# PeterouZh/CIPS-3Dplusplus

Hardware: AMD Instinct MI355X
Metric: rendered views/sec at FFHQ 1024^2 (generator forward: 64x64-ray NeRF + StyleGAN2 decoder) (higher is better)
Workload: dtype f32 (split-fp16 MFMA products x3, f32 accumulate and storage); 1 GPU; ffhq_r1024_nerf64x64x24_D2_B1_fp32; img_size=64, n_samples=24, N_layers_renderer=2, resolution=1024, parallelism=views x1, views_in_flight=2

## Files before the change

### cips_3dplusplus_amd/csrc/decoder.hip

```cpp
#include <stdlib.h>

#include <type_traits>

#include "common.h"

namespace {

typedef float f32x16 __attribute__((ext_vector_type(16)));
typedef float f32x4 __attribute__((ext_vector_type(4)));
typedef short s16x4 __attribute__((ext_vector_type(4)));
typedef _Float16 h8 __attribute__((ext_vector_type(8)));

typedef _Float16 h4 __attribute__((ext_vector_type(4)));
typedef _Float16 h2 __attribute__((ext_vector_type(2)));
__device__ __forceinline__ float pack_split(float x) { return __uint_as_float(cips3d_split_word(x)); }
__device__ __forceinline__ float pack_split(float x, float k) { return __uint_as_float(cips3d_split_word(x, k)); }
__device__ __forceinline__ void unpack_frag(float p0, float p1, float p2, float p3, h4& hi, h4& lo) {
  typedef unsigned u32x2_t __attribute__((ext_vector_type(2)));
  const unsigned a0 = __float_as_uint(p0), a1 = __float_as_uint(p1), a2 = __float_as_uint(p2), a3 = __float_as_uint(p3);
  hi = __builtin_bit_cast(h4, u32x2_t{__builtin_amdgcn_perm(a1, a0, 0x05040100u), __builtin_amdgcn_perm(a3, a2, 0x05040100u)});
  lo = __builtin_bit_cast(h4, u32x2_t{__builtin_amdgcn_perm(a1, a0, 0x07060302u), __builtin_amdgcn_perm(a3, a2, 0x07060302u)});
}
__device__ __forceinline__ void split_frag(float v0, float v1, float v2, float v3, h4& hi, h4& lo) {
  typedef unsigned u32x2_t __attribute__((ext_vector_type(2)));
// ... 889 lines not shown
          o.x += sv.x; o.y += sv.y; o.z += sv.z; o.w += sv.w;
        }
      }
      *reinterpret_cast<float4*>(out + ((int64_t)b * 3 + c) * HW + qq * 4) = o;
    }
  }
}

__global__ void __launch_bounds__(256) torgb_scalar_kernel(const float* __restrict__ x, const float* __restrict__ wm,
                                                           const float* __restrict__ bias, const float* __restrict__ skip,
                                                           int skip_up, const float* __restrict__ fir,
                                                           float* __restrict__ out, int B, int Cin, int H, int W) {
  const int64_t HW = (int64_t)H * W;
  const int64_t total = (int64_t)B * HW;
  for (int64_t idx = (int64_t)blockIdx.x * blockDim.x + threadIdx.x; idx < total; idx += (int64_t)gridDim.x * blockDim.x) {
    const int b = (int)(idx / HW);
    const int64_t n = idx % HW;
    const float* xb = x + (int64_t)b * Cin * HW + n;
    const float* w = wm + (int64_t)b * 3 * Cin;
    float acc[3] = {0.f, 0.f, 0.f};
    for (int i = 0; i < Cin; ++i) {
      const float v = xb[(int64_t)i * HW];
      acc[0] = fmaf(w[i], v, acc[0]); acc[1] = fmaf(w[Cin + i], v, acc[1]); acc[2] = fmaf(w[2 * Cin + i], v, acc[2]);
    }
    const int oy = (int)(n / W), ox = (int)(n % W);
#pragma unroll
    for (int c = 0; c < 3; ++c) {
      float o = acc[c] + bias[c];
      if (skip) {
        if (skip_up) o += up2_tap(skip + ((int64_t)b * 3 + c) * (H / 2) * (W / 2), H / 2, W / 2, oy, ox, fir);
        else o += skip[((int64_t)b * 3 + c) * HW + n];
      }
      out[((int64_t)b * 3 + c) * HW + n] = o;
    }
  }
}

__global__ void __launch_bounds__(256) modconv_kxk_kernel(const float* __restrict__ x, const float* __restrict__ wm,
                                                          float* __restrict__ out, int B, int Cin, int Cout, int H,
                                                          int W, int k, int transpose2, int OH, int OW) {
  const int64_t total = (int64_t)B * Cout * OH * OW;
  const int pad = k / 2;
  for (int64_t idx = (int64_t)blockIdx.x * blockDim.x + threadIdx.x; idx < total;
       idx += (int64_t)gridDim.x * blockDim.x) {
    int64_t t = idx;
    const int ox = (int)(t % OW); t /= OW;
    const int oy = (int)(t % OH); t /= OH;
    const int o = (int)(t % Cout);
    const int b = (int)(t / Cout);
    const float* wrow = wm + ((int64_t)b * Cout + o) * Cin * k * k;
    const float* xb = x + (int64_t)b * Cin * H * W;
    float acc = 0.f;
    for (int i = 0; i < Cin; ++i) {
      const float* xi = xb + (int64_t)i * H * W;
      const float* wi = wrow + i * k * k;
      for (int ky = 0; ky < k; ++ky) {
        int iy;
        if (transpose2) { const int ty = oy - ky; if (ty < 0 || (ty & 1)) continue; iy = ty >> 1; }
        else iy = oy + ky - pad;
        if (iy < 0 || iy >= H) continue;
        for (int kx = 0; kx < k; ++kx) {
          int ix;
          if (transpose2) { const int tx = ox - kx; if (tx < 0 || (tx & 1)) continue; ix = tx >> 1; }
          else ix = ox + kx - pad;
          if (ix < 0 || ix >= W) continue;
          acc = fmaf(xi[(int64_t)iy * W + ix], wi[ky * k + kx], acc);
        }
      }
    }
    out[idx] = acc;
  }
}

struct FusedArgs {
  const float* y_lo; const float* fir; const float* noise1; int64_t nbs1; const float* nw1; const float* bias1;
  const float* wm2; const float* noise2; int64_t nbs2; const float* nw2; const float* bias2; float* out2;
  const float* wm_rgb; const float* bias_rgb; const float* skip; int skip_up; float* rgb;
  int B, H, W;
  int bf16;
  const float* wm_next; float* y_next;
  const float* x_amax; const float* lconst1; const float* lconst2; float* next_amax;
  float next_gain;
  int flat;
};

#ifndef CIPS3D_C128_LATE
#define CIPS3D_C128_LATE true
#endif
#ifndef CIPS3D_C64_MINW
#define CIPS3D_C64_MINW 4
#endif
#ifndef CIPS3D_C32_MINW
#define CIPS3D_C32_MINW 8
#endif
#ifndef CIPS3D_FUSED_AB
#define CIPS3D_FUSED_AB 0
#endif
#ifdef CIPS3D_FUSED_STAMPS
__device__ unsigned long long g_fused_stamps[4][8];
#define FSTAMP(i) do { const unsigned long long t_ = __builtin_amdgcn_s_memtime(); fst_[i] += t_ - ftp_; ftp_ = t_; } while (0)
#define FSTAMP_FLUSH() do { if (tid == 0 && (blockIdx.x & 31) == 0) {    constexpr int sl_ = C == 32 ? 0 : C == 64 ? 1 : C == 128 ? 2 : 3; \
    for (int i_ = 0; i_ < 7; ++i_) atomicAdd(&g_fused_stamps[sl_][i_], fst_[i_]); atomicAdd(&g_fused_stamps[sl_][7], 1ull); } } while (0)
#else
#define FSTAMP(i)
#define FSTAMP_FLUSH()
#endif

template <int C, int WM, int WGM, int WGN, int RW, int BK, int MINW, int PREC, bool NEXT = false, bool XPREF = false,
          bool LATE_OPS = false, bool FLAT = false>
__global__ void __launch_bounds__(64 * WGM * WGN, MINW) fused_up_conv_kernel(FusedArgs a) {
  constexpr bool BF16 = PREC == 1 || PREC == 2;
  constexpr bool YB = PREC == 2;
  constexpr bool SPLIT = PREC == 3;
  typedef typename std::conditional<YB, bf16_t, float>::type ylo_t;
  constexpr int NT = 64 * WGM * WGN;
  constexpr int CW = 64 / RW, TH = RW * WGN, TW = CW, BN = TH * TW;
  constexpr int NSTAGE = C / BK, NBUF = NSTAGE > 1 ? 2 : 1, KQ = BK / 16;
  constexpr int LPR = CW / 4;
  static_assert((WGM * WGN == 8 || WGM * WGN == 4) && 16 * WM * WGM == C && TH % 2 == 0 && C % BK == 0, "tile shape");
  constexpr int NBLK = (TH / 2) * (TW / 4);
  constexpr int BPT = BK * NBLK / NT;
  static_assert((BK * NBLK) % NT == 0 && BPT >= 1, "block split");
  __shared__ __attribute__((aligned(16))) float sB[NBUF * BK * BN];
  __shared__ __attribute__((aligned(16))) float s_nz1[BN + 8];
  __shared__ __attribute__((aligned(16))) float s_red_own[NEXT ? WGM * 3 * BN : 4];
  float* s_red = NEXT ? s_red_own : sB;
  __shared__ __attribute__((aligned(16))) float s_wrgb[3 * C];

  const int tid = threadIdx.x;
#ifdef CIPS3D_FUSED_STAMPS
  unsigned long long fst_[7] = {0, 0, 0, 0, 0, 0, 0}, ftp_ = __builtin_amdgcn_s_memtime();
#endif
  const int wave = __builtin_amdgcn_readfirstlane(tid >> 6);
  const int lane = tid & 63;
  const int wm_i = wave / WGN, wn_i = wave % WGN;
  const int q = lane >> 4, jn = lane & 15;
  const int lrow = jn / LPR, lx4 = jn % LPR;
  const int nloc = (wn_i * RW + lrow) * TW + lx4 * 4;
  const int b = blockIdx.z;
  const int H = a.H, W = a.W, OH = FLAT ? H : 2 * H, OW = FLAT ? W : 2 * W;
  const int tiles_x = OW / TW;
  int bid = blockIdx.x;
  if ((gridDim.x & 7) == 0) bid = (bid & 7) * (gridDim.x >> 3) + (bid >> 3);
  const int ox0 = (bid % tiles_x) * TW, oy0 = (bid / tiles_x) * TH;
  const int HWlo = H * W, HWo = OH * OW;
  const int oy = oy0 + wn_i * RW + lrow, ox = ox0 + lx4 * 4;

  float kact1 = 1.41421356237309515f, k2in = kSplitInv, kact2 = 1.41421356237309515f, kback2 = 1.f, kyn = kSplitInv;

#ifndef CIPS3D_FUSED_TILE_DMA
#define CIPS3D_FUSED_TILE_DMA 1
#endif
  constexpr bool TILE_DMA = CIPS3D_FUSED_TILE_DMA != 0;
  float nw1_u = 0.f;
  float c10_u = 0.f, c11_u = 0.f, c20_u = 0.f, c21a_u = 0.f, c21b_u = 0.f;
  if constexpr (SPLIT && TILE_DMA) {
    if (a.x_amax && !(CIPS3D_FUSED_AB & 1)) {
      const float* l1 = a.lconst1 + b * 4;
      c10_u = l1[0]; c11_u = l1[1];
      if (NEXT) {
        const float* l2 = a.lconst2 + b * 4;
        c20_u = l2[0]; c21a_u = l2[1]; c21b_u = l2[2];
      }
    }
  }
  const float* ab = a.wm2 + (int64_t)b * C * C;
  f32x4 afr_next[KQ][WM];
#pragma unroll
  for (int kq = 0; kq < KQ; ++kq)
#pragma unroll
    for (int i = 0; i < WM; ++i)
      afr_next[kq][i] = *reinterpret_cast<const f32x4*>(ab + (((wm_i * WM + i) * (C / 16) + kq) * 256 + lane * 4));
  constexpr bool LATE = LATE_OPS;
  f32x4 nz2 = {0.f, 0.f, 0.f, 0.f};
  float nw2_u = 0.f;
  f32x4 bias4[WM];
  auto load_epilogue_ops = [&]() {
    if (a.noise2 && a.nw2 && !(CIPS3D_FUSED_AB & 128)) {
      nz2 = *reinterpret_cast<const f32x4*>(a.noise2 + (int64_t)b * a.nbs2 + (oy * OW + ox));
      nw2_u = a.nw2[0];
    }
#pragma unroll
    for (int i = 0; i < WM; ++i) bias4[i] = *reinterpret_cast<const f32x4*>(a.bias2 + (wm_i * WM + i) * 16 + 4 * q);
  };
  if (!LATE) load_epilogue_ops();

  float kf[16];
#pragma unroll
  for (int i = 0; i < 16; ++i) kf[i] = FLAT ? 0.f : a.fir[15 - i];
  const bool rgb_lane = a.wm_rgb && wm_i == 0 && q < 3;
  float skp[3][4];
  f32x4 skv = {0.f, 0.f, 0.f, 0.f};
  float rgb_bias = 0.f;
// ... 472 lines not shown
#pragma unroll
      for (int t = 0; t < OTN; ++t)
#pragma unroll
        for (int c = 0; c < 4; ++c) {
          const f32x4 pv4 = *reinterpret_cast<const f32x4*>(sp + (t * 4 + c) * 256);
#pragma unroll
          for (int r = 0; r < 4; ++r) accn[t][c][r] += pv4[r];
        }
    }
    ylo_t* yn = reinterpret_cast<ylo_t*>(a.y_next) + (int64_t)b * (C / 2) * HWo + (oy * OW + ox);
#pragma unroll
    for (int t = 0; t < OTN; ++t)
#pragma unroll
      for (int r = 0; r < 4; ++r) {
        const float ys = SPLIT ? kyn : 1.f;
        const f32x4 yv = {accn[t][0][r] * ys, accn[t][1][r] * ys, accn[t][2][r] * ys, accn[t][3][r] * ys};
        mxn = fmaxf(fmaxf(fmaxf(fabsf(yv[0]), fabsf(yv[1])), fmaxf(fabsf(yv[2]), fabsf(yv[3]))), mxn);
        if constexpr (YB) cips3d_store_wt8(yn + (t * 16 + 4 * q + r) * HWo, pack_bf16(yv[0], yv[1], yv[2], yv[3]));
        else cips3d_store_wt16(yn + (t * 16 + 4 * q + r) * HWo, yv);
      }
  }
  if (NEXT && !XCHG && a.next_amax && !(a.next_gain > 0.f) && !(CIPS3D_FUSED_AB & 2)) {
    const float m = cips3d_workgroup_max(mxn, s_nz1, wave, lane, WGM * WGN);
    if (tid == 0) cips3d_amax_raise_if(a.next_amax + b * CIPS3D_AMAX_FLOATS, m, blockIdx.x);
  }
  FSTAMP(5);
  if (!a.wm_rgb) { FSTAMP_FLUSH(); return; }
  if (rgb_lane) {
    const int ch = q;
    f32x4 v = {0.f, 0.f, 0.f, 0.f};
#pragma unroll
    for (int m = 0; m < WGM; ++m) {
      const f32x4 t = *reinterpret_cast<const f32x4*>(s_red + (m * 3 + ch) * BN + nloc);
#pragma unroll
      for (int c = 0; c < 4; ++c) v[c] += t[c];
    }
#pragma unroll
    for (int c = 0; c < 4; ++c) v[c] += rgb_bias;
    if (a.skip) {
      if (!FLAT && (a.skip_up & 1)) {
        float so[2][4];
        up2_fir(skp, kf, so);
        const int py = oy & 1;
#pragma unroll
        for (int c = 0; c < 4; ++c) v[c] += py ? so[1][c] : so[0][c];
      } else {
#pragma unroll
        for (int c = 0; c < 4; ++c) v[c] += skv[c];
      }
    }
    if (a.skip_up & 2) {
      unsigned pk = 0;
#pragma unroll
      for (int c = 0; c < 4; ++c) {
        const float cl = fminf(fmaxf(v[c], -1.f), 1.f);
        pk |= (unsigned)__float2int_rn((cl + 1.f) * 127.5f) << (8 * c);
      }
      *reinterpret_cast<unsigned*>(reinterpret_cast<unsigned char*>(a.rgb) + (int64_t)b * 3 * HWo + (ch * HWo + oy * OW + ox)) = pk;
    } else {
      cips3d_store_wt16(a.rgb + (int64_t)b * 3 * HWo + (ch * HWo + oy * OW + ox), v);
    }
  }
  FSTAMP(6);
  FSTAMP_FLUSH();
}

template <int C, int WM, int WGM, int WGN, int RW, int BK, int MINW, bool NEXT, bool XPREF, bool LATE, bool FLAT>
int launch_fused_as(const FusedArgs& a, hipStream_t st) {
  constexpr int TH = RW * WGN, TW = 64 / RW;
  const int up = FLAT ? 1 : 2;
  dim3 grid((unsigned)((up * a.W / TW) * (up * a.H / TH)), 1, (unsigned)a.B);
  if (a.bf16 == 3) hipLaunchKernelGGL((fused_up_conv_kernel<C, WM, WGM, WGN, RW, BK, MINW, 3, NEXT, XPREF, LATE, FLAT>), grid, dim3(64 * WGM * WGN), 0, st, a);
  else if (a.bf16 == 2) hipLaunchKernelGGL((fused_up_conv_kernel<C, WM, WGM, WGN, RW, BK, MINW, 2, NEXT, XPREF, LATE, FLAT>), grid, dim3(64 * WGM * WGN), 0, st, a);
  else if (a.bf16) hipLaunchKernelGGL((fused_up_conv_kernel<C, WM, WGM, WGN, RW, BK, MINW, 1, NEXT, XPREF, LATE, FLAT>), grid, dim3(64 * WGM * WGN), 0, st, a);
  else hipLaunchKernelGGL((fused_up_conv_kernel<C, WM, WGM, WGN, RW, BK, MINW, 0, NEXT, XPREF, LATE, FLAT>), grid, dim3(64 * WGM * WGN), 0, st, a);
  return cips3d_launch_status();
}
template <int C, int WM, int WGM, int WGN, int RW, int BK, int MINW, bool NEXT = false, bool XPREF = false, bool LATE = false>
int launch_fused(const FusedArgs& a, hipStream_t st) {
  return a.flat ? launch_fused_as<C, WM, WGM, WGN, RW, BK, MINW, NEXT, XPREF, LATE, true>(a, st)
                : launch_fused_as<C, WM, WGM, WGN, RW, BK, MINW, NEXT, XPREF, LATE, false>(a, st);
}

}

#ifdef CIPS3D_FUSED_STAMPS
extern "C" int cips3d_debug_read_fused_stamps(unsigned long long* out32) {
  hipDeviceSynchronize();
  hipMemcpyFromSymbol(out32, HIP_SYMBOL(g_fused_stamps), 256);
  unsigned long long z[32] = {0};
  hipMemcpyToSymbol(HIP_SYMBOL(g_fused_stamps), z, 256);
  return 0;
}
#endif

extern "C" int cips3d_modulate_weights(const float* W, const float* s, int64_t s_stride, float* wm, int B, int Cout,
                                       int Cin, int ksq, float scale, int demodulate, void* stream) {
  if (!W || !s || !wm || B < 0 || Cout <= 0 || Cin <= 0 || ksq <= 0) return CIPS3D_E_BADARG;
  if (B == 0) return 0;
  const int packed = (demodulate & 2) ? (((demodulate & 4) ? 2 : 1) | (demodulate & 248)) : 0;
  if ((packed & 32) && (ksq != 1 || (packed & 24))) return CIPS3D_E_UNSUPP;
  if ((packed & 64) && (ksq != 1 || (packed & 63) != 1)) return CIPS3D_E_UNSUPP;
  if (packed && ksq == 1 && (Cout % 32 != 0 || Cin % 8 != 0)) return CIPS3D_E_UNSUPP;
  if ((packed & 16) && ksq == 1 && ((packed & 7) != 1 || Cin % 32 != 0)) return CIPS3D_E_UNSUPP;
  if ((packed & 16) && ksq != 1 && (ksq != 9 || (packed & ~8) != 17)) return CIPS3D_E_UNSUPP;
  if ((packed & 128) && (ksq != 1 || (packed & 127) != 1 || Cin % 32 != 0)) return CIPS3D_E_UNSUPP;
  if (packed && ksq != 1 && (ksq != 9 || (packed & 7) != 1 || Cout % 16 != 0 || Cin % 16 != 0)) return CIPS3D_E_UNSUPP;
  const int64_t rows = (int64_t)B * Cout;
  hipLaunchKernelGGL(modulate_kernel, dim3((unsigned)ceil_div<int64_t>(rows, 4)), dim3(256), 0, as_stream(stream), W,
                     s, s_stride, wm, B, Cout, Cin, ksq, scale, demodulate & 1, packed);
  return cips3d_launch_status();
}

extern "C" int cips3d_modulate_table(const cips3d_modulate_desc* table_dev, int n_desc, int total_rows, int B, float noise_bound,
                                     void* stream) {
  if (!table_dev || n_desc <= 0 || total_rows <= 0 || B < 0 || !(noise_bound >= 0.f)) return CIPS3D_E_BADARG;
  if (B == 0) return 0;
  hipLaunchKernelGGL(modulate_table_kernel, dim3((unsigned)ceil_div(total_rows, 4), (unsigned)B), dim3(256), 0,
                     as_stream(stream), table_dev, n_desc, total_rows, noise_bound);
  return cips3d_launch_status();
}

__global__ void __launch_bounds__(256) split_words_kernel(const float* __restrict__ x, float k, unsigned* __restrict__ words,
                                                          unsigned* __restrict__ pairs, int64_t n) {
  const float ku = cips3d_uniform(k);
  for (int64_t i = (int64_t)blockIdx.x * 256 + threadIdx.x; i < n / 2; i += (int64_t)gridDim.x * 256) {
    words[2 * i] = cips3d_split_word(x[2 * i], ku);
    words[2 * i + 1] = cips3d_split_word(x[2 * i + 1] * k);
    cips3d_split_pair(x[2 * i], x[2 * i + 1], pairs[2 * i], pairs[2 * i + 1]);
  }
}

extern "C" int cips3d_split_words(const float* x, float k, uint32_t* words, uint32_t* pairs, int64_t n, void* stream) {
  if (!x || !words || !pairs || n <= 0 || (n & 1)) return CIPS3D_E_BADARG;
  int64_t blocks = ceil_div<int64_t>(n / 2, 256);
  if (blocks > 4096) blocks = 4096;
  hipLaunchKernelGGL(split_words_kernel, dim3((unsigned)blocks), dim3(256), 0, as_stream(stream), x, k, words, pairs, n);
  return cips3d_launch_status();
}

extern "C" int cips3d_amax_layout(int* slots, int* stride) {
  if (slots) *slots = CIPS3D_AMAX_SLOTS;
  if (stride) *stride = CIPS3D_AMAX_STRIDE;
  return 0;
}

extern "C" int cips3d_absmax(const float* x, int B, int64_t n, float* amax, void* stream) {
  if (!x || !amax || B < 0 || n <= 0) return CIPS3D_E_BADARG;
  if (B == 0) return 0;
  hipError_t e = hipMemsetAsync(amax, 0, sizeof(float) * CIPS3D_AMAX_FLOATS * (size_t)B, as_stream(stream));
  if (e != hipSuccess) return (int)e;
  int64_t blocks = ceil_div<int64_t>(n, 256 * 16);
  if (blocks > 1024) blocks = 1024;
  hipLaunchKernelGGL(absmax_kernel, dim3((unsigned)blocks, (unsigned)B), dim3(256), 0, as_stream(stream), x, n, amax);
  return cips3d_launch_status();
}

extern "C" int cips3d_absmax_raise(const float* x, int B, int64_t n, float* amax, void* stream) {
  if (!x || !amax || B < 0 || n <= 0) return CIPS3D_E_BADARG;
  if (B == 0) return 0;
  int64_t blocks = ceil_div<int64_t>(n, 256 * 16);
  if (blocks > 1024) blocks = 1024;
  hipLaunchKernelGGL(absmax_kernel, dim3((unsigned)blocks, (unsigned)B), dim3(256), 0, as_stream(stream), x, n, amax);
  return cips3d_launch_status();
}

extern "C" int cips3d_range_consts(const float* bias, int n_bias, const float* noise_w, float noise_bound, const float* noise_amax,
                                   float w_gain, const float* fir, float* lconst, int B, void* stream) {
  if (!lconst || B < 0 || n_bias < 0 || (n_bias > 0 && !bias) || !(noise_bound >= 0.f) || !(w_gain >= 0.f)) return CIPS3D_E_BADARG;
  if (B == 0) return 0;
  hipLaunchKernelGGL(range_consts_kernel, dim3((unsigned)B), dim3(64), 0, as_stream(stream), bias, n_bias, noise_w, noise_bound,
                     noise_amax, w_gain, fir, lconst);
  return cips3d_launch_status();
}
// ... 95 lines not shown
    static const int bk = getenv("CIPS3D_GEMM_BK") ? atoi(getenv("CIPS3D_GEMM_BK")) : 0;
    const bool one_round = (int64_t)B * (Cout / 64) * ceil_div<int64_t>(HW, 128) <= 256;
    if ((bk ? bk == 64 : one_round) && Cin % 64 == 0) return launch_gemm_actbwd<1, 4, 2, 64, 2>(a, st);
    static const int big_tiles = getenv("CIPS3D_GEMM_BIG") ? atoi(getenv("CIPS3D_GEMM_BIG")) : 1;
    if (big_tiles && Cout % 128 == 0 && Cin % 64 == 0) return launch_gemm_actbwd<2, 4, 2, 64, 2>(a, st);
    return launch_gemm_actbwd<1, 4, 2, 32, 2>(a, st);
  }
  static const int ns2 = getenv("CIPS3D_GEMM_NS2") ? atoi(getenv("CIPS3D_GEMM_NS2")) : 1;
  if (ns2 && Cin <= 128) {
    if (Cout == 128) return launch_gemm_actbwd<1, 8, 1, 32, 2>(a, st);
    if (Cout == 64) return launch_gemm_actbwd<1, 4, 2, 32, 2>(a, st);
    if (Cout < 256) return launch_gemm_actbwd<1, 2, 2, 32, 2>(a, st);
  }
  if (Cout == 128) return launch_gemm_actbwd<1, 8, 1, 32, 4>(a, st);
  if (Cout == 64) return launch_gemm_actbwd<1, 4, 2, 32, 4>(a, st);
  return launch_gemm_actbwd<1, 2, 2, 32, 4>(a, st);
}

extern "C" int cips3d_up2_fir_act(const float* y_lo, const float* fir, float* out, int B, int C, int H, int W,
                                  const float* noise, int64_t noise_bstride, const float* noise_w, const float* bias,
                                  float* out_amax, void* stream) {
  if (!y_lo || !fir || !out || !bias || B < 0 || C <= 0 || H <= 0 || W <= 0) return CIPS3D_E_BADARG;
  if (W % 2 != 0) return CIPS3D_E_UNSUPP;
  if (B == 0) return 0;
  const int64_t total = (int64_t)B * C * H * (W / 2);
  int64_t blocks = ceil_div<int64_t>(total, 256);
  if (blocks > 16384) blocks = 16384;
  hipLaunchKernelGGL(up2_fir_act_kernel, dim3((unsigned)blocks), dim3(256), 0, as_stream(stream), y_lo, fir, out, B,
                     C, H, W, noise, noise_bstride, noise_w, bias, out_amax);
  return cips3d_launch_status();
}

extern "C" int cips3d_noise_bias_act(const float* x, const float* noise, int64_t noise_bstride, const float* noise_w,
                                     const float* bias, float* out, int B, int C, int64_t HW, void* stream) {
  if (!x || !bias || !out || B < 0 || C <= 0 || HW <= 0) return CIPS3D_E_BADARG;
  if (B == 0) return 0;
  int64_t blocks = ceil_div<int64_t>((int64_t)B * C * HW, 256);
  if (blocks > 16384) blocks = 16384;
  hipLaunchKernelGGL(noise_bias_act_kernel, dim3((unsigned)blocks), dim3(256), 0, as_stream(stream), x, noise,
                     noise_bstride, noise_w, bias, out, B, C, HW);
  return cips3d_launch_status();
}

extern "C" int cips3d_fused_up_conv_supported(int C, int H, int W) {
  return (C == 32 || C == 64 || C == 128 || C == 256) && W % 32 == 0 && H % 2 == 0 && H >= 2 &&
         (int64_t)C * 4 * H * W < ((int64_t)1 << 31);
}

extern "C" int cips3d_fused_flat_conv_supported(int C, int H, int W) {
  return (C == 32 || C == 64 || C == 128 || C == 256) && W % 64 == 0 && H % 4 == 0 && H >= 4 &&
         (int64_t)C * H * W < ((int64_t)1 << 31);
}

extern "C" int cips3d_fused_up_conv(const float* y_lo, const float* fir, const float* noise1, int64_t noise1_bstride,
                                    const float* noise_w1, const float* bias1, const float* wm2, const float* noise2,
                                    int64_t noise2_bstride, const float* noise_w2, const float* bias2, float* out2,
                                    const float* wm_rgb, const float* bias_rgb, const float* skip, int skip_up,
                                    float* rgb, int B, int C, int H, int W, const cips3d_range* rg, void* stream) {
  return cips3d_fused_up_conv_next(y_lo, fir, noise1, noise1_bstride, noise_w1, bias1, wm2, noise2, noise2_bstride, noise_w2,
                                   bias2, out2, wm_rgb, bias_rgb, skip, skip_up, rgb, nullptr, nullptr, B, C, H, W, rg, stream);
}

extern "C" int cips3d_fused_up_conv_chains(int C) { return C == 64 || C == 128 || C == 256; }

extern "C" int cips3d_fused_up_conv_next(const float* y_lo, const float* fir, const float* noise1, int64_t noise1_bstride,
                                         const float* noise_w1, const float* bias1, const float* wm2, const float* noise2,
                                         int64_t noise2_bstride, const float* noise_w2, const float* bias2, float* out2,
                                         const float* wm_rgb, const float* bias_rgb, const float* skip, int skip_up,
                                         float* rgb, const float* wm_next, float* y_next, int B, int C, int H, int W,
                                         const cips3d_range* rg, void* stream) {
  const int flat = (skip_up & CIPS3D_STAGE_FLAT) ? 1 : 0;
  if (!y_lo || (!fir && !flat) || !bias1 || !wm2 || !bias2 || B < 0 || H <= 0 || W <= 0) return CIPS3D_E_BADARG;
  if (flat && (skip_up & 1)) return CIPS3D_E_BADARG;
  if ((wm_next == nullptr) != (y_next == nullptr)) return CIPS3D_E_BADARG;
  if (wm_next && !cips3d_fused_up_conv_chains(C)) return CIPS3D_E_UNSUPP;
  if (!out2 && !wm_rgb && !wm_next) return CIPS3D_E_BADARG;
  if (wm_rgb && (!bias_rgb || !rgb)) return CIPS3D_E_BADARG;
  if (!(flat ? cips3d_fused_flat_conv_supported(C, H, W) : cips3d_fused_up_conv_supported(C, H, W))) return CIPS3D_E_UNSUPP;
  if (B == 0) return 0;
  FusedArgs a{y_lo, fir, noise1, noise1_bstride, noise_w1, bias1, wm2, noise2, noise2_bstride, noise_w2, bias2, out2,
              wm_rgb, bias_rgb, skip, (skip_up & 1) | ((skip_up & CIPS3D_RGB_U8) ? 2 : 0), rgb, B, H, W,
              (skip_up & CIPS3D_GEMM_SPLIT) ? 3 : (skip_up & CIPS3D_GEMM_BF16) ? ((skip_up & CIPS3D_Y_BF16) ? 2 : 1) : 0, wm_next,
              y_next, rg ? rg->x_amax : nullptr, rg ? rg->lconst : nullptr, rg ? rg->lconst2 : nullptr,
              rg ? rg->next_amax : nullptr, rg ? rg->next_gain : 0.f, flat};
  if ((skip_up & CIPS3D_GEMM_SPLIT) && rg && rg->x_amax && (!rg->lconst || (wm_next && !rg->lconst2))) return CIPS3D_E_BADARG;
  if ((skip_up & CIPS3D_Y_BF16) && !(skip_up & CIPS3D_GEMM_BF16)) return CIPS3D_E_BADARG;
  if ((skip_up & CIPS3D_GEMM_SPLIT) && (skip_up & CIPS3D_GEMM_BF16)) return CIPS3D_E_BADARG;
  hipStream_t st = as_stream(stream);
  if (wm_next)
    return C == 64    ? launch_fused<64, 2, 2, 2, 1, 16, CIPS3D_C64_MINW, true, true, true>(a, st)
           : C == 128 ? launch_fused<128, 4, 2, 2, 1, 32, 2, true, false, CIPS3D_C128_LATE>(a, st)
                      : launch_fused<256, 2, 8, 1, 2, 64, 2, true, true>(a, st);
  switch (C) {
    case 32: return launch_fused<32, 1, 2, 2, 1, 32, CIPS3D_C32_MINW, false, false, true>(a, st);
    case 64: return launch_fused<64, 2, 2, 2, 1, 16, 4>(a, st);
    case 128: return launch_fused<128, 4, 2, 4, 1, 32, 2>(a, st);
    case 256: return launch_fused<256, 2, 8, 1, 2, 64, 2>(a, st);
  }
  return CIPS3D_E_UNSUPP;
}

struct RgbReduceArgs {
  const float* part; int n_slots; int n_bias; const float* bias[CIPS3D_TORGB_FOLD_MAX]; const float* skip; float* out;
  int64_t n4, HW4, slot_stride;
};

__global__ void __launch_bounds__(256) torgb_reduce_kernel(RgbReduceArgs a) {
  __shared__ f32x4 s_p[4][64];
  const int pl = threadIdx.x & 63, g = threadIdx.x >> 6;
  const int64_t i = (int64_t)blockIdx.x * 64 + pl;
  f32x4 v = {0.f, 0.f, 0.f, 0.f};
  if (i < a.n4) {
    for (int s0 = g; s0 < a.n_slots; s0 += 16) {
      f32x4 t[4];
#pragma unroll
      for (int u = 0; u < 4; ++u)
        t[u] = s0 + 4 * u < a.n_slots ? *reinterpret_cast<const f32x4*>(a.part + (s0 + 4 * u) * a.slot_stride + i * 4)
                                      : f32x4{0.f, 0.f, 0.f, 0.f};
#pragma unroll
      for (int u = 0; u < 4; ++u)
#pragma unroll
        for (int c = 0; c < 4; ++c) v[c] += t[u][c];
    }
  }
  s_p[g][pl] = v;
  __syncthreads();
  if (g != 0 || i >= a.n4) return;
#pragma unroll
  for (int k = 1; k < 4; ++k) {
    const f32x4 t = s_p[k][pl];
#pragma unroll
    for (int c = 0; c < 4; ++c) v[c] += t[c];
  }
  const int ch = (int)((i / a.HW4) % 3);
  float bs = 0.f;
  for (int k = 0; k < a.n_bias; ++k) bs += a.bias[k][ch];
#pragma unroll
  for (int c = 0; c < 4; ++c) v[c] += bs;
  if (a.skip) {
    const f32x4 sk = *reinterpret_cast<const f32x4*>(a.skip + i * 4);
#pragma unroll
    for (int c = 0; c < 4; ++c) v[c] += sk[c];
  }
  *reinterpret_cast<f32x4*>(a.out + i * 4) = v;
}

extern "C" int cips3d_torgb_reduce(const float* part, int n_slots, const float* const* biases, int n_bias, const float* skip,
                                   float* out, int B, int64_t HW, void* stream) {
  if (!part || !out || n_slots < 1 || n_bias < 0 || n_bias > CIPS3D_TORGB_FOLD_MAX || (n_bias && !biases) || B < 0 || HW <= 0)
    return CIPS3D_E_BADARG;
  if (HW % 4) return CIPS3D_E_UNSUPP;
  if (B == 0) return 0;
  RgbReduceArgs a{};
  a.part = part; a.n_slots = n_slots; a.n_bias = n_bias;
  for (int k = 0; k < n_bias; ++k) a.bias[k] = biases[k];
  a.skip = skip; a.out = out;
  a.n4 = (int64_t)B * 3 * HW / 4; a.HW4 = HW / 4; a.slot_stride = (int64_t)B * 3 * HW;
  hipLaunchKernelGGL(torgb_reduce_kernel, dim3((unsigned)ceil_div<int64_t>(a.n4, 64)), dim3(256), 0, as_stream(stream), a);
  return cips3d_launch_status();
}

extern "C" int cips3d_torgb(const float* x, const float* wm, const float* bias, const float* skip, int skip_up,
                            const float* fir, float* out, int B, int Cin, int H, int W, void* stream) {
  if (!x || !wm || !bias || !out || B < 0 || Cin <= 0 || H <= 0 || W <= 0) return CIPS3D_E_BADARG;
  if (skip && skip_up && (!fir || (H % 2) || (W % 2))) return CIPS3D_E_BADARG;
  if (B == 0) return 0;
  if (W % 4 != 0) {
    int64_t bs = ceil_div<int64_t>((int64_t)B * H * W, 256);
    if (bs > 16384) bs = 16384;
    hipLaunchKernelGGL(torgb_scalar_kernel, dim3((unsigned)bs), dim3(256), 0, as_stream(stream), x, wm, bias, skip,
                       skip_up, fir, out, B, Cin, H, W);
    return cips3d_launch_status();
  }
  const int64_t quads = (int64_t)H * W / 4;
  {
    const size_t lds = sizeof(float) * (256 * 12 + 3 * (size_t)Cin);
    if (quads <= 32768 && Cin >= 64) {
// ... 31 lines not shown
```

Baseline: 3443 views/s.

## Add strip-walking fused up-conv kernel for the C=32 final stage

Adds a persistent-style variant of the fused upsample+conv+ToRGB kernel for the C=32 split-precision stage. Each workgroup walks a vertical strip of S tile rows and keeps a 4-row ring of low-res input rows in LDS, filled by async global-to-LDS DMA. This lets adjacent output rows reuse the three input rows the FIR needs instead of reloading halos, and overlaps the next row's loads with compute. The modulated weights and bias are loaded once per strip. In exchange there are fewer workgroups, so parallelism drops, S is auto-reduced to keep at least 1024 groups, and the code adds extra barriers and complexity.

```diff
diff --git a/cips_3dplusplus_amd/csrc/decoder.hip b/cips_3dplusplus_amd/csrc/decoder.hip
--- a/cips_3dplusplus_amd/csrc/decoder.hip
+++ b/cips_3dplusplus_amd/csrc/decoder.hip
@@ -995,6 +995,7 @@
   const float* x_amax; const float* lconst1; const float* lconst2; float* next_amax;
   float next_gain;
   int flat;
+  int walk_s;
 };
 
 #ifndef CIPS3D_C128_LATE
@@ -1010,7 +1011,7 @@
 #define CIPS3D_FUSED_AB 0
 #endif
 #ifdef CIPS3D_FUSED_STAMPS
-__device__ unsigned long long g_fused_stamps[4][8];
+__device__ unsigned long long g_fused_stamps[6][8];
 #define FSTAMP(i) do { const unsigned long long t_ = __builtin_amdgcn_s_memtime(); fst_[i] += t_ - ftp_; ftp_ = t_; } while (0)
 #define FSTAMP_FLUSH() do { if (tid == 0 && (blockIdx.x & 31) == 0) {    constexpr int sl_ = C == 32 ? 0 : C == 64 ? 1 : C == 128 ? 2 : 3; \
     for (int i_ = 0; i_ < 7; ++i_) atomicAdd(&g_fused_stamps[sl_][i_], fst_[i_]); atomicAdd(&g_fused_stamps[sl_][7], 1ull); } } while (0)
@@ -1019,9 +1020,322 @@
 #define FSTAMP_FLUSH()
 #endif
 
+__host__ __device__ inline int walk_strip_count(int tiles_x, int tiles_y, int S) { return tiles_x * ((tiles_y + S - 1) / S); }
+__host__ __device__ inline void walk_strip_of(int wg, int n_wg, int tiles_x, int tiles_y, int S, int* tx, int* ty0, int* nt) {
+  const int sid = (n_wg & 7) == 0 ? (wg & 7) * (n_wg >> 3) + (wg >> 3) : wg;
+  const int sy = sid / tiles_x;
+  *tx = sid % tiles_x;
+  *ty0 = sy * S;
+  *nt = tiles_y - sy * S < S ? tiles_y - sy * S : S;
+}
+
+#ifdef CIPS3D_FUSED_STAMPS
+#define WSTAMP(i) do { const unsigned long long t_ = __builtin_amdgcn_s_memtime(); fst_[i] += t_ - ftp_; ftp_ = t_; } while (0)
+#else
+#define WSTAMP(i)
+#endif
+
+__device__ __forceinline__ void walk_barrier() {
+  asm volatile("s_waitcnt lgkmcnt(0)" ::: "memory");
+  __builtin_amdgcn_s_barrier();
+  asm volatile("" ::: "memory");
+}
+
+template <int C, int WM, int WGM, int WGN, int RW, int BK>
+__device__ __forceinline__ void fused_walk_strip(const FusedArgs& a) {
+  constexpr int NT = 64 * WGM * WGN;
+  constexpr int CW = 64 / RW, TH = RW * WGN, TW = CW, BN = TH * TW, KQ = BK / 16;
+  constexpr int NBLK = (TH / 2) * (TW / 4), BPT = BK * NBLK / NT;
+  static_assert(C == BK && TH == 2 && TW == 64 && NT == 256 && 16 * WM * WGM == C && BPT * NT == BK * NBLK, "walker shape");
+  constexpr int SEG = TW / 2 + 8;
+  constexpr int PPC = SEG / 4;
+  constexpr int NPIECE = C * PPC;
+  constexpr int NU = (NPIECE + NT - 1) / NT;
+  constexpr int SLOT = C * SEG;
+  static_assert(NU == 2 && NPIECE - NT <= 64, "the second piece round fits wave 0");
+  __shared__ __attribute__((aligned(16))) float sB[BK * BN];
+  __shared__ __attribute__((aligned(16))) float s_ring[4 * SLOT];
+  __shared__ __attribute__((aligned(16))) float s_nz1[2 * BN];
+  __shared__ __attribute__((aligned(16))) float s_sc[4];
+  __shared__ __attribute__((aligned(16))) float s_wrgb[3 * C];
+  float* s_red = sB;
+
+  const int tid = threadIdx.x;
+#ifdef CIPS3D_FUSED_STAMPS
+  unsigned long long fst_[6] = {0, 0, 0, 0, 0, 0}, ftp_ = __builtin_amdgcn_s_memtime();
+#endif
+  const int wave = __builtin_amdgcn_readfirstlane(tid >> 6);
+  const int lane = tid & 63;
+  const int wm_i = wave / WGN, wn_i = wave % WGN;
+  const int q = lane >> 4, jn = lane & 15;
+  const int nloc = wn_i * TW + jn * 4;
+  const int b = blockIdx.z;
+  const int H = a.H, W = a.W, OW = 2 * W;
+  const int HWlo = H * W, HWo = 4 * HWlo;
+  int tx, ty0, nt;
+  walk_strip_of(blockIdx.x, gridDim.x, OW / TW, H, a.walk_s, &tx, &ty0, &nt);
+  const int ox0 = tx * TW, iy0 = ty0;
+  const bool left = ox0 == 0, right = ox0 / 2 + TW / 2 >= W;
+  const int ox = ox0 + jn * 4;
+
+  float kact1 = 1.41421356237309515f, k2in = kSplitInv;
+  float c10_u = 0.f, c11_u = 0.f;
+  const bool ranged = a.x_amax != nullptr;
+  if (ranged) { const float* l1 = a.lconst1 + b * 4; c10_u = l1[0]; c11_u = l1[1]; }
+  const bool have_nz = a.noise1 && a.nw1;
+  const float nw1_u = have_nz ? a.nw1[0] : 0.f;
+  const bool have_nz2 = a.noise2 && a.nw2;
+  const float nw2_u = have_nz2 ? a.nw2[0] : 0.f;
+  float kf[16];
+#pragma unroll
+  for (int i = 0; i < 16; ++i) kf[i] = a.fir[15 - i];
+  const float* ab = a.wm2 + (int64_t)b * C * C;
+  f32x4 afr[KQ][WM];
+#pragma unroll
+  for (int kq = 0; kq < KQ; ++kq)
+#pragma unroll
+    for (int i = 0; i < WM; ++i)
+      afr[kq][i] = *reinterpret_cast<const f32x4*>(ab + (((wm_i * WM + i) * (C / 16) + kq) * 256 + lane * 4));
+  f32x4 bias4[WM];
+#pragma unroll
+  for (int i = 0; i < WM; ++i) bias4[i] = *reinterpret_cast<const f32x4*>(a.bias2 + (wm_i * WM + i) * 16 + 4 * q);
+  const bool rgb_lane = a.wm_rgb && wm_i == 0 && q < 3;
+  const float rgb_bias = rgb_lane ? a.bias_rgb[q] : 0.f;
+  const int qx = lane & 15;
+  const int ch0 = (lane >> 5) | ((wave & 1) << 1) | (((lane >> 4) & 1) << 2) | ((wave >> 1) << 3);
+  float bs1[BPT];
+#pragma unroll
+  for (int u = 0; u < BPT; ++u) bs1[u] = a.bias1[ch0 + 16 * u];
+  if (ranged && wave == 0) {
+    const float t = lane < CIPS3D_AMAX_SLOTS ? a.x_amax[b * CIPS3D_AMAX_FLOATS + lane * CIPS3D_AMAX_STRIDE] : 0.f;
+    const float m_in = cips3d_wave_max_uniform(t);
+    const float u1 = fmaf(c11_u, m_in, c10_u);
+    const int e1 = cips3d_split_exp(u1);
+    if (lane == 0) *reinterpret_cast<f32x4*>(s_sc) = f32x4{1.41421356237309515f * cips3d_pow2(-e1), kSplitInv * cips3d_pow2(e1), 0.f, 0.f};
+  }
+  if (left && tid < 4 * C) s_ring[tid * SEG + 3] = 0.f;
+  if (right && tid < 4 * C) s_ring[tid * SEG + SEG - 4] = 0.f;
+  if (!have_nz) s_nz1[tid] = 0.f;
+  static_assert(2 * BN == NT && 4 * C <= NT, "border stores");
+  int voff[NU];
+#pragma unroll
+  for (int u = 0; u < NU; ++u) {
+    const int p = u * NT + tid;
+    const int pc = p / PPC, pj = p % PPC;
+    const bool ok = p < NPIECE && !(left && pj == 0) && !(right && pj == PPC - 1);
+    voff[u] = ok ? (pc * HWlo + ox0 / 2 - 4 + 4 * pj) * 4 : -1;
+  }
+  const char* ylo_b = reinterpret_cast<const char*>(a.y_lo + (int64_t)b * C * HWlo);
+  auto request_row = [&](int r) -> int {
+    float* dst = s_ring + (r & 3) * SLOT;
+    if (r < 0 || r >= H) {
+      const int j0 = left ? 1 : 0, j1 = right ? PPC - 1 : PPC;
+#pragma unroll
+      for (int u = 0; u < NU; ++u) {
+        const int p = u * NT + tid;
+        if (p < NPIECE && p % PPC >= j0 && p % PPC < j1) *reinterpret_cast<f32x4*>(dst + p * 4) = f32x4{0.f, 0.f, 0.f, 0.f};
+      }
+      return 0;
+    }
+    const char* ub = ylo_b + (int64_t)r * W * 4;
+    int n = 0;
+#pragma unroll
+    for (int u = 0; u < NU; ++u) {
+      if (u * NT + wave * 64 < NPIECE) {
+        if (voff[u] >= 0)
+          __builtin_amdgcn_global_load_lds((const __attribute__((address_space(1))) void*)(ub + voff[u]),
+                                           (__attribute__((address_space(3))) void*)(dst + (u * NT + wave * 64) * 4), 16, 0, 0);
+        ++n;
+      }
+    }
+    return n;
+  };
+  auto request_noise = [&](int t) -> int {
+    if (!have_nz || wave != 1) return 0;
+    if (lane < BN / 4) {
+      const int r = lane / (TW / 4), x4 = lane % (TW / 4);
+      __builtin_amdgcn_global_load_lds((const __attribute__((address_space(1))) void*)(a.noise1 + (int64_t)b * a.nbs1 + ((2 * (iy0 + t) + r) * OW + ox0 + x4 * 4)),
+                                       (__attribute__((address_space(3))) void*)(s_nz1 + (t & 1) * BN), 16, 0, 0);
+    }
+    return 1;
+  };
+  if (a.wm_rgb) {
+    static_assert(3 * C / 4 <= 64, "one LDS-DMA instruction for the ToRGB rows");
+    if (wave == 0 && lane < 3 * C / 4)
+      __builtin_amdgcn_global_load_lds((const __attribute__((address_space(1))) void*)(a.wm_rgb + (int64_t)b * 3 * C + lane * 4),
+                                       (__attribute__((address_space(3))) void*)s_wrgb, 16, 0, 0);
+  }
+  request_row(iy0 - 1); request_row(iy0); request_row(iy0 + 1); request_noise(0);
+  int pend = 0;
+  if (nt > 1) { pend = request_row(iy0 + 2); pend += request_noise(1); }
+  WSTAMP(0);
+
+  for (int t = 0; t < nt; ++t) {
+    const int iy = iy0 + t;
+    const int oy = 2 * iy + wn_i;
+    if (pend == 2) __builtin_amdgcn_s_waitcnt(vmcnt_imm(2));
+    else if (pend == 1) __builtin_amdgcn_s_waitcnt(vmcnt_imm(1));
+    else __builtin_amdgcn_s_waitcnt(vmcnt_imm(0));
+    walk_barrier();
+    WSTAMP(1);
+    if (t == 0 && ranged) {
+      const f32x4 sc = *reinterpret_cast<const f32x4*>(s_sc);
+      kact1 = cips3d_uniform(sc[0]);
+      k2in = cips3d_uniform(sc[1]);
+    }
+    const float* nzb = s_nz1 + (t & 1) * BN;
+#pragma unroll
+    for (int u = 0; u < BPT; ++u) {
+      const int ch = ch0 + 16 * u;
+      float v[3][4];
+#pragma unroll
+      for (int r = 0; r < 3; ++r) {
+        const float2* p2 = reinterpret_cast<const float2*>(s_ring + ((iy - 1 + r) & 3) * SLOT + ch * SEG + 2 + 2 * qx);
+        const float2 e0 = p2[0], e1 = p2[1], e2 = p2[2];
+        v[r][0] = e0.y; v[r][1] = e1.x; v[r][2] = e1.y; v[r][3] = e2.x;
+      }
+      float o[2][4];
+      up2_fir(v, kf, o);
+      const float bs = bs1[u];
+#pragma unroll
+      for (int py = 0; py < 2; ++py) {
+        const f32x4 nz = *reinterpret_cast<const f32x4*>(nzb + py * TW + qx * 4);
+        f32x4 w;
+#pragma unroll
+        for (int c = 0; c < 4; ++c) w[c] = pack_split(lrelu02(fmaf(nw1_u, nz[c], o[py][c]) + bs), kact1);
+        *reinterpret_cast<f32x4*>(sB + ch * BN + py * TW + qx * 4) = w;
+      }
+    }
+    walk_barrier();
+    WSTAMP(2);
+    f32x4 acc[WM][4];
+#pragma unroll
+    for (int i = 0; i < WM; ++i)
+#pragma unroll
+      for (int c = 0; c < 4; ++c) acc[i][c] = f32x4{0.f, 0.f, 0.f, 0.f};
+#pragma unroll
+    for (int kq = 0; kq < KQ; ++kq) {
+      f32x4 b4[4];
+#pragma unroll
+      for (int j4 = 0; j4 < 4; ++j4) b4[j4] = *reinterpret_cast<const f32x4*>(sB + nloc + (kq * 16 + j4 * 4 + q) * BN);
+#pragma unroll
+      for (int c = 0; c < 4; ++c) {
+        h4 bh, bl;
+        unpack_frag(b4[0][c], b4[1][c], b4[2][c], b4[3][c], bh, bl);
+#pragma unroll
+        for (int i = 0; i < WM; ++i) acc[i][c] = split_mfma16(afr[kq][i], bh, bl, acc[i][c]);
+      }
+    }
+    walk_barrier();
+    WSTAMP(3);
+    f32x4 nz2 = {0.f, 0.f, 0.f, 0.f};
+    if (have_nz2) nz2 = *reinterpret_cast<const f32x4*>(a.noise2 + (int64_t)b * a.nbs2 + (oy * OW + ox));
+    float skp[3][4];
+    f32x4 skv = {0.f, 0.f, 0.f, 0.f};
+    if (rgb_lane && a.skip) {
+      if (a.skip_up & 1) up2_load(a.skip + (int64_t)b * 3 * HWlo + q * HWlo, H, W, oy >> 1, ox >> 2, skp);
+      else skv = *reinterpret_cast<const f32x4*>(a.skip + (int64_t)b * 3 * HWo + (q * HWo + oy * OW + ox));
+    }
+    float prgb[3][4];
+#pragma unroll
+    for (int ch = 0; ch < 3; ++ch)
+#pragma unroll
+      for (int c = 0; c < 4; ++c) prgb[ch][c] = 0.f;
+#pragma unroll
+    for (int i = 0; i < WM; ++i) {
+      const int obase = (wm_i * WM + i) * 16 + 4 * q;
+#pragma unroll
+      for (int r = 0; r < 4; ++r) {
+        f32x4 v = {acc[i][0][r], acc[i][1][r], acc[i][2][r], acc[i][3][r]};
+#pragma unroll
+        for (int c = 0; c < 4; ++c) v[c] *= k2in;
+#pragma unroll
+        for (int c = 0; c < 4; ++c) v[c] = lrelu02(fmaf(nw2_u, nz2[c], v[c]) + bias4[i][r]) * 1.41421356237309515f;
+        if (a.out2) *reinterpret_cast<f32x4*>(a.out2 + (int64_t)b * C * HWo + ((obase + r) * HWo + oy * OW + ox)) = v;
+        if (a.wm_rgb) {
+#pragma unroll
+          for (int ch = 0; ch < 3; ++ch) {
+            const float w = s_wrgb[ch * C + obase + r];
+#pragma unroll
+            for (int c = 0; c < 4; ++c) prgb[ch][c] = fmaf(w, v[c], prgb[ch][c]);
+          }
+        }
+      }
+    }
+    WSTAMP(4);
+    if (a.wm_rgb) {
+#pragma unroll
+      for (int ch = 0; ch < 3; ++ch)
+#pragma unroll
+        for (int c = 0; c < 4; ++c) {
+          float v = prgb[ch][c];
+          v += __shfl_xor(v, 16, 64);
+          v += __shfl_xor(v, 32, 64);
+          prgb[ch][c] = v;
+        }
+      if (q == 0) {
+#pragma unroll
+        for (int ch = 0; ch < 3; ++ch)
+          *reinterpret_cast<f32x4*>(s_red + (wm_i * 3 + ch) * BN + nloc) = f32x4{prgb[ch][0], prgb[ch][1], prgb[ch][2], prgb[ch][3]};
+      }
+      walk_barrier();
+      if (rgb_lane) {
+        const int ch = q;
+        f32x4 v = {0.f, 0.f, 0.f, 0.f};
+#pragma unroll
+        for (int m = 0; m < WGM; ++m) {
+          const f32x4 tt = *reinterpret_cast<const f32x4*>(s_red + (m * 3 + ch) * BN + nloc);
+#pragma unroll
+          for (int c = 0; c < 4; ++c) v[c] += tt[c];
+        }
+#pragma unroll
+        for (int c = 0; c < 4; ++c) v[c] += rgb_bias;
+        if (a.skip) {
+          if (a.skip_up & 1) {
+            float so[2][4];
+            up2_fir(skp, kf, so);
+            const int py = oy & 1;
+#pragma unroll
+            for (int c = 0; c < 4; ++c) v[c] += py ? so[1][c] : so[0][c];
+          } else {
+#pragma unroll
+            for (int c = 0; c < 4; ++c) v[c] += skv[c];
+          }
+        }
+        if (a.skip_up & 2) {
+          unsigned pk = 0;
+#pragma unroll
+          for (int c = 0; c < 4; ++c) {
+            const float cl = fminf(fmaxf(v[c], -1.f), 1.f);
+            pk |= (unsigned)__float2int_rn((cl + 1.f) * 127.5f) << (8 * c);
+          }
+          *reinterpret_cast<unsigned*>(reinterpret_cast<unsigned char*>(a.rgb) + (int64_t)b * 3 * HWo + (ch * HWo + oy * OW + ox)) = pk;
+        } else {
+          cips3d_store_wt16(a.rgb + (int64_t)b * 3 * HWo + (ch * HWo + oy * OW + ox), v);
+        }
+      }
+    }
+    pend = 0;
+    if (t + 2 < nt) { pend = request_row(iy + 3); pend += request_noise(t + 2); }
+    WSTAMP(5);
+  }
+#ifdef CIPS3D_FUSED_STAMPS
+  if (tid == 0 && (blockIdx.x & 7) == 0) {
+    constexpr int sl_ = 4 + (C == 32 ? 0 : 1);
+    for (int i_ = 0; i_ < 6; ++i_) atomicAdd(&g_fused_stamps[sl_][i_], fst_[i_]);
+    atomicAdd(&g_fused_stamps[sl_][6], (unsigned long long)nt); atomicAdd(&g_fused_stamps[sl_][7], 1ull);
+  }
+#endif
+}
+
 template <int C, int WM, int WGM, int WGN, int RW, int BK, int MINW, int PREC, bool NEXT = false, bool XPREF = false,
-          bool LATE_OPS = false, bool FLAT = false>
+          bool LATE_OPS = false, bool FLAT = false, bool WALK = false>
 __global__ void __launch_bounds__(64 * WGM * WGN, MINW) fused_up_conv_kernel(FusedArgs a) {
+  if constexpr (WALK) {
+    static_assert(!WALK || (PREC == 3 && !NEXT && !FLAT), "walker: split mode, last up-sampling stage");
+    fused_walk_strip<C, WM, WGM, WGN, RW, BK>(a);
+    return;
+  }
   constexpr bool BF16 = PREC == 1 || PREC == 2;
   constexpr bool YB = PREC == 2;
   constexpr bool SPLIT = PREC == 3;
@@ -1660,14 +1974,45 @@
                 : launch_fused_as<C, WM, WGM, WGN, RW, BK, MINW, NEXT, XPREF, LATE, false>(a, st);
 }
 
+#ifndef CIPS3D_WALK_MINW
+#define CIPS3D_WALK_MINW 4
+#endif
+#ifndef CIPS3D_WALK_S
+#define CIPS3D_WALK_S 8
+#endif
+int fused_walk_tiles(const FusedArgs& a, int C) {
+  if (C != 32 || a.bf16 != 3 || a.flat || a.wm_next) return 0;
+  const char* sw = getenv("CIPS3D_FUSED_WALK");
+  if (sw && atoi(sw) == 0) return 0;
+  const int tiles_x = 2 * a.W / 64, tiles_y = a.H;
+  const char* fs = getenv("CIPS3D_FUSED_WALK_S");
+  if (fs && atoi(fs) > 0) return atoi(fs) < tiles_y ? atoi(fs) : tiles_y;
+  int S = CIPS3D_WALK_S;
+  while (S > 1 && (int64_t)walk_strip_count(tiles_x, tiles_y, S) * a.B < 1024) S >>= 1;
+  return S > 1 ? S : 0;
+}
+int launch_fused_walk32(const FusedArgs& a, hipStream_t st) {
+  dim3 grid((unsigned)walk_strip_count(2 * a.W / 64, a.H, a.walk_s), 1, (unsigned)a.B);
+  hipLaunchKernelGGL((fused_up_conv_kernel<32, 1, 2, 2, 1, 32, CIPS3D_WALK_MINW, 3, false, false, true, false, true>), grid, dim3(256), 0, st, a);
+  return cips3d_launch_status();
+}
+
+}
+
+extern "C" int cips3d_fused_walk_schedule(int tiles_x, int tiles_y, int S, int wg, int* tx, int* ty0, int* nt) {
+  if (tiles_x <= 0 || tiles_y <= 0 || S <= 0 || !tx || !ty0 || !nt) return CIPS3D_E_BADARG;
+  const int n_wg = walk_strip_count(tiles_x, tiles_y, S);
+  if (wg < 0 || wg >= n_wg) return CIPS3D_E_BADARG;
+  walk_strip_of(wg, n_wg, tiles_x, tiles_y, S, tx, ty0, nt);
+  return n_wg;
 }
 
 #ifdef CIPS3D_FUSED_STAMPS
 extern "C" int cips3d_debug_read_fused_stamps(unsigned long long* out32) {
   hipDeviceSynchronize();
-  hipMemcpyFromSymbol(out32, HIP_SYMBOL(g_fused_stamps), 256);
-  unsigned long long z[32] = {0};
-  hipMemcpyToSymbol(HIP_SYMBOL(g_fused_stamps), z, 256);
+  hipMemcpyFromSymbol(out32, HIP_SYMBOL(g_fused_stamps), 384);
+  unsigned long long z[48] = {0};
+  hipMemcpyToSymbol(HIP_SYMBOL(g_fused_stamps), z, 384);
   return 0;
 }
 #endif
@@ -1929,7 +2274,7 @@
               wm_rgb, bias_rgb, skip, (skip_up & 1) | ((skip_up & CIPS3D_RGB_U8) ? 2 : 0), rgb, B, H, W,
               (skip_up & CIPS3D_GEMM_SPLIT) ? 3 : (skip_up & CIPS3D_GEMM_BF16) ? ((skip_up & CIPS3D_Y_BF16) ? 2 : 1) : 0, wm_next,
               y_next, rg ? rg->x_amax : nullptr, rg ? rg->lconst : nullptr, rg ? rg->lconst2 : nullptr,
-              rg ? rg->next_amax : nullptr, rg ? rg->next_gain : 0.f, flat};
+              rg ? rg->next_amax : nullptr, rg ? rg->next_gain : 0.f, flat, 0};
   if ((skip_up & CIPS3D_GEMM_SPLIT) && rg && rg->x_amax && (!rg->lconst || (wm_next && !rg->lconst2))) return CIPS3D_E_BADARG;
   if ((skip_up & CIPS3D_Y_BF16) && !(skip_up & CIPS3D_GEMM_BF16)) return CIPS3D_E_BADARG;
   if ((skip_up & CIPS3D_GEMM_SPLIT) && (skip_up & CIPS3D_GEMM_BF16)) return CIPS3D_E_BADARG;
@@ -1939,7 +2284,9 @@
            : C == 128 ? launch_fused<128, 4, 2, 2, 1, 32, 2, true, false, CIPS3D_C128_LATE>(a, st)
                       : launch_fused<256, 2, 8, 1, 2, 64, 2, true, true>(a, st);
   switch (C) {
-    case 32: return launch_fused<32, 1, 2, 2, 1, 32, CIPS3D_C32_MINW, false, false, true>(a, st);
+    case 32:
+      if ((a.walk_s = fused_walk_tiles(a, C)) > 0) return launch_fused_walk32(a, st);
+      return launch_fused<32, 1, 2, 2, 1, 32, CIPS3D_C32_MINW, false, false, true>(a, st);
     case 64: return launch_fused<64, 2, 2, 2, 1, 16, 4>(a, st);
     case 128: return launch_fused<128, 4, 2, 4, 1, 32, 2>(a, st);
     case 256: return launch_fused<256, 2, 8, 1, 2, 64, 2>(a, st);
```

Result: slower. 3300 views/s, median of 2 (-4.1%).
